# William-Mou/WasmEdge

Measured on AMD Instinct MI355X. Metric: aggregate Wasm instrs/sec at 64K instances, 1/2/4/8 GPUs vs host-core interp, higher is better.
Workload: dtype i32; 1 GPU; C2 BLAKE3 compression loop (configs[1]); instances_per_gpu=65536, instances=65536, parallelism=instance-sharded, 1 process per GPU, compiled_runs=11, engine=compiled-runs+simt/vgpr-frames, granule=4, iters=1000

## Files before the change

### wasmedge_amd/csrc/batch_kernel.hip

```cpp
#include <hip/hip_runtime.h>
#include <stdint.h>

#include <mutex>
#include <vector>

#include "dbc.h"
#include "kparams.h"


#include "dbc_ops.h"
#include "tc.h"
#include "tc_slots.h"

extern "C" __global__ void wb_tc_holder_kernel() {
  asm volatile("s_endpgm\n"
#include "tc_blob.inc"
               ::: "s60", "s61", "s62", "s63", "s64", "s65", "s66", "s67", "s68", "s69",
               "s70", "s71", "s72", "s73", "s74", "s75", "s76", "s77", "s78", "s79", "s80",
               "s81", "s82", "s83", "s84", "s85", "s86", "s87", "s88", "s89", "s90", "s91",
               "s92", "s93", "s94", "s95", "v104", "v105", "v106", "v107", "v108", "v109", "v110", "v111",
               "v112", "v113", "v114", "v115", "v116", "v117", "v118", "v119", "v120",
               "v121", "v122", "v123", "v124", "v125", "v126", "v127", "vcc", "memory");
}
extern "C" __global__ void __launch_bounds__(256) wb_vf_holder_kernel() {
// ... 124 lines not shown
      "v_mov_b32 v105, %[pages]\n\t" \
      "v_mov_b32 v106, %[mlo]\n\t" \
      "v_mov_b32 v107, %[mhi]\n\t" \
      "v_mov_b32 v102, %[gsp]\n\t" \
      "v_mov_b32 v101, %[hwm]\n\t" \
      "v_mov_b32 v103, %[stk]\n\t" \
      "v_mov_b32 v99, %[msh]\n\t" \
      "v_add_u32_e32 v100, 6, v99\n\t" \
      "v_mov_b32 v92, %[vpc]\n\t" \
      "v_mov_b32 v93, 0\n\t" \
      "s_mov_b32 s93, %[slds]\n\t" \
      "v_mov_b32 v94, %[llo]\n\t" \
      "v_mov_b32 v95, %[lhi]\n\t" \
      "v_mov_b32 v96, %[glo]\n\t" \
      "v_mov_b32 v97, %[ghi]\n\t" \
      "s_mov_b32 s94, %[vsync]\n\t" \
      "s_mov_b32 s95, %[low]\n\t" \
      "s_mov_b32 s98, %[xlo]\n\t" \
      "s_mov_b32 s99, %[xhi]\n\t" \
      "s_mov_b64 exec, s[96:97]\n\t" \
      "s_getpc_b64 s[66:67]\n" \
      "Ltc_ret_%=:\n\t" \
      "s_add_u32 s66, s66, Ltc_back_%= - Ltc_ret_%=\n\t" \
      "s_addc_u32 s67, s67, 0\n\t" \
      "s_getpc_b64 s[68:69]\n\t" \
      "s_add_u32 s68, s68, wb_vf_entry@rel32@lo+4\n\t" \
      "s_addc_u32 s69, s69, wb_vf_entry@rel32@hi+12\n\t" \
      "s_setpc_b64 s[68:69]\n" \
      "Ltc_back_%=:\n\t" \
      "s_lshr_b32 %[npc], s62, 5\n\t" \
      "s_mov_b32 %[cnt], s65\n\t" \
      "s_mov_b32 %[why], s92\n\t" \
      "s_mov_b32 %[noth], s63\n\t" \
      "s_mov_b32 %[nlow], s95\n\t" \
      "s_mov_b64 %[ngrp], s[74:75]\n\t" \
      "v_mov_b32 %[gsp], v102\n\t" \
      "v_mov_b32 %[glo], v96\n\t" \
      "v_mov_b32 %[ghi], v97\n\t" \
      "v_mov_b32 %[vpc], v92\n\t" \
      "v_mov_b32 %[vcnt], v93\n\t" \
      "v_mov_b32 %[hwm], v101\n\t" \
      "s_mov_b64 exec, %[ex]" \
       \
      : [npc] "=&s"(npc), [cnt] "=&s"(cnt), [why] "=&s"(why), [noth] "=&s"(noth), [nlow] "=&s"(nlow), \
        [ngrp] "=&s"(ngrp), [gsp] "+v"(gsp), [hwm] "+v"(hwm), [glo] "+v"(glo), [ghi] "+v"(ghi), \
        [vpc] "+v"(vpc), [vcnt] "=&v"(vcnt) \
      : [clo] "s"(clo), [chi] "s"(chi), [pc] "s"(pc), [oth] "s"(oth), [lim] "s"(lim), [fr] "v"(fr), \
        [pages] "v"(pages), [mlo] "v"(mlo), [mhi] "v"(mhi), [stk] "v"(stk), [msh] "s"(msh), \
        [slds] "s"(slds), [vsync] "s"(vsync), [low] "s"(lw), [llo] "s"(llo), [lhi] "s"(lhi), \
        [all] "s"(all), [grp] "s"(grp), [ex] "s"(ex), [xlo] "s"(xlo), [xhi] "s"(xhi) \
      : "s60", "s61", "s62", "s63", "s64", "s65", "s66", "s67", "s68", "s69", "s70", "s71", \
        "s72", "s73", "s74", "s75", "s76", "s77", "s78", "s79", "s80", "s81", "s82", "s83", \
        "s84", "s85", "s86", "s87", "s88", "s89", "s90", "s91", "s92", "s93", "s94", "s95", "s96", "s97", \
        "s98", "s99", \
        "v92", "v93", "v94", "v98", "v95", "v96", "v97", "v99", "v100", "v101", "v102", "v103", "v104", "v105", "v106", "v107", "v108", "v109", "v110", "v111", "v112", "v113", \
        "v114", "v115", "v116", "v117", "v118", "v119", "v120", "v121", "v122", "v123", \
        "v124", "v125", "v126", "v127", "vcc", "scc", "memory", ##__VA_ARGS__);
#define TC_VREGS "v128", "v129", "v130", "v131", "v132", "v133", "v134", "v135", "v136", "v137", \
  "v138", "v139", "v140", "v141", "v142", "v143", "v144", "v145", "v146", "v147", "v148", "v149", \
  "v150", "v151", "v152", "v153", "v154", "v155", "v156", "v157", "v158", "v159", "v160", "v161", \
  "v162", "v163", "v164", "v165", "v166", "v167", "v168", "v169", "v170", "v171", "v172", "v173", \
  "v174", "v175", "v176", "v177", "v178", "v179", "v180", "v181", "v182", "v183", "v184", "v185", \
  "v186", "v187", "v188", "v189", "v190", "v191", "v192", "v193", "v194", "v195", "v196", "v197", \
  "v198", "v199", "v200", "v201", "v202", "v203", "v204", "v205", "v206", "v207", "v208", "v209", \
  "v210", "v211", "v212", "v213", "v214", "v215", "v216", "v217", "v218", "v219", "v220", "v221", \
  "v222", "v223", "v224", "v225", "v226", "v227", "v228", "v229", "v230", "v231", "v232", "v233", \
  "v234", "v235", "v236", "v237", "v238", "v239", "v240", "v241", "v242", "v243", "v244", "v245", \
  "v246", "v247", "v248", "v249", "v250", "v251", "v252", "v253", "v254", "v255"
struct SimtOut {
  uint64_t grp;
  uint32_t oth, low, vpc, vcnt;
};
template <bool VF>
__device__ __forceinline__ uint32_t tc_run(const void *tcode, uint32_t pc, uint32_t other, uint32_t low,
                                           uint32_t fr, uint32_t pages, const uint32_t *mem, uint32_t g,
                                           uint32_t &gsp, uint32_t &hwm, uint32_t stk, uint32_t slds,
                                           uint32_t vsync, uint64_t &gas, uint64_t gas_limit,
                                           uint32_t *ncnt, uint32_t *reason, uint32_t lim,
                                           SimtOut *so = nullptr, uint64_t all = 0, uint64_t grp = 0,
                                           uint32_t vpc = 0, uint64_t xbase = 0) {
  uint32_t npc, cnt, why;
  uint32_t glo = (uint32_t)gas, ghi = (uint32_t)(gas >> 32);
  const uint32_t llo = __builtin_amdgcn_readfirstlane((uint32_t)gas_limit);
  const uint32_t lhi = __builtin_amdgcn_readfirstlane((uint32_t)(gas_limit >> 32));
  const uint32_t oth = __builtin_amdgcn_readfirstlane(other >= (1u << 26) ? 0xFFFFFFFFu : other << 5);
  const uint32_t lw = __builtin_amdgcn_readfirstlane(low >= (1u << 26) ? 0xFFFFFFFFu : low << 5);
  const uint64_t m = (uint64_t)(uintptr_t)mem;
  const uint32_t msh = 2u + g;
  const uint32_t mlo = (uint32_t)m, mhi = (uint32_t)(m >> 32);
  const uint64_t cp = (uint64_t)(uintptr_t)tcode;
  const uint32_t clo = (uint32_t)cp, chi = (uint32_t)(cp >> 32);
  pc = __builtin_amdgcn_readfirstlane(pc);
  if constexpr (VF) {
    const uint64_t ex = __builtin_amdgcn_read_exec();
    if (!so) all = grp = ex;
    const uint32_t xlo = __builtin_amdgcn_readfirstlane((uint32_t)xbase);
    const uint32_t xhi = __builtin_amdgcn_readfirstlane((uint32_t)(xbase >> 32));
    uint32_t noth, nlow, vcnt;
    uint64_t ngrp;
    TC_RUN_VF_ASM(TC_VREGS);
    if (so) *so = SimtOut{ngrp, noth, nlow, vpc, vcnt};
  } else {
    TC_RUN_ASM("wb_tc_entry");
  }
  gas = (uint64_t)glo | ((uint64_t)ghi << 32);
  *ncnt = cnt;
  *reason = why;
// ... 832 lines not shown
```

### wasmedge_amd/csrc/jit.cpp

```cpp
#include "jit.h"

#include <algorithm>
#include <cctype>
#include <cstdarg>
#include <cstdio>
#include <cstdlib>
#include <functional>
#include <map>

#include "frontend.h"
#include "jit_int.h"
#include "tc_slots.h"

namespace wb {
using namespace jit;

namespace {

constexpr uint32_t kMinRun = 3;
constexpr uint32_t kMaxRun = 1500;
constexpr uint32_t kMaxBrTable = 32;

const char *const PAGES = "v105", *const MEM = "v[106:107]", *const HWM = "v101";
const char *const A0 = "v108", *const A1 = "v109", *const AP = "v[108:109]";
const char *const B0 = "v110", *const B1 = "v111", *const BP = "v[110:111]";
const char *const R0 = "v114", *const R1 = "v115", *const RP = "v[114:115]";
const char *const W0 = "v116", *const WP = "v[116:117]";
const char *const X0 = "v118", *const X1 = "v119", *const XP = "v[118:119]";
const char *const Y0 = "v120", *const Y1 = "v121";
const char *const Z0 = "v126", *const Z1 = "v127", *const ZP = "v[126:127]";
const char *const T2 = "s[74:75]";

uint16_t op_of(const DInstr &I) { return uint16_t(I.w0 & 0x7FFFu); }

bool is_store_op(uint16_t op) {
  return op == OP_ST8 || op == OP_ST16 || op == OP_ST32 || op == OP_ST64 || op == OP_ST128;
}

uint32_t mem_bytes(uint16_t op) {
  switch (op) {
    case OP_LD8S32: case OP_LD8U32: case OP_LD8S64: case OP_LD8U64: case OP_ST8: return 1;
    case OP_LD16S32: case OP_LD16U32: case OP_LD16S64: case OP_LD16U64: case OP_ST16: return 2;
    case OP_LD32: case OP_LD32S64: case OP_LD32U64: case OP_ST32: return 4;
    case OP_LD64: case OP_ST64: return 8;
    case OP_LD128: case OP_ST128: return 16;
    default: return 0;
  }
}

bool load_wide_op(uint16_t op) {
  return op == OP_LD8S64 || op == OP_LD8U64 || op == OP_LD16S64 || op == OP_LD16U64 ||
         op == OP_LD32S64 || op == OP_LD32U64 || op == OP_LD64;
}
uint16_t xmop(const DInstr &I) {
  const uint16_t op = uint16_t(I.w0 & 0x7FFFu);
  return op == OP_XLD || op == OP_XST ? uint16_t(I.w2 >> 16) : uint16_t(0);
}
bool is_xfer(uint16_t op) { return op == OP_CALL || op == OP_RET; }
bool is_branch_op(uint16_t op) {
  return op == OP_JMP || op == OP_BR_IF || op == OP_BR_UNLESS || (op >= OP_BR_EQ && op <= OP_BR_GE_U_I);
}
bool ends_run(uint16_t op) { return is_xfer(op) || is_branch_op(op) || op == OP_BR_TABLE || op == OP_TAIL_CALL; }

struct JitTarget {
  const Program &P;
  uint32_t glog;
  const JitCost *cost;
  const std::vector<uint32_t> *xinfo;
  uint32_t xlog;
  uint32_t mem_pages;
};

struct RunIndex {
  std::map<uint32_t, size_t> start;
  std::map<uint32_t, uint32_t> fentry;
  uint32_t ncode;
  RunIndex(const Program &P, const std::vector<JitRun> &runs) : ncode(uint32_t(P.code.size())) {
    for (size_t k = 0; k < runs.size(); k++) start.emplace(runs[k].pc, k);
    for (uint32_t f = 0; f < P.funcs.size(); f++)
      if (!P.funcs[f].imported) fentry[P.funcs[f].entry_pc] = f;
  }
  bool has(uint32_t pc) const { return start.count(pc) != 0; }
  size_t at(uint32_t pc) const { return start.find(pc)->second; }
  int64_t func_of(uint32_t pc) const {
// ... 3425 lines not shown
  return fp;
}

bool jit::recursive(const Program &P) {
  const RunIndex ix(P, {});
  auto func_of = [&](uint32_t pc) { return ix.func_of(pc); };
  const size_t nf = P.funcs.size();
  std::vector<std::vector<uint32_t>> g(nf);
  for (uint32_t pc = 0; pc < P.code.size(); pc++) {
    const uint16_t o = op_of(P.code[pc]);
    if (o == OP_CALL_INDIRECT || o == OP_TAIL_CALL_INDIRECT) return true;
    if (o != OP_CALL && o != OP_TAIL_CALL) continue;
    const int64_t a = func_of(pc), b = func_of(P.code[pc].w3);
    if (a < 0 || b < 0) continue;
    if (a == b) return true;
    g[size_t(a)].push_back(uint32_t(b));
  }
  std::vector<uint8_t> st(nf, 0);
  std::function<bool(uint32_t)> dfs = [&](uint32_t f) -> bool {
    st[f] = 1;
    for (uint32_t t : g[f]) {
      if (st[t] == 1) return true;
      if (st[t] == 0 && dfs(t)) return true;
    }
    st[f] = 2;
    return false;
  };
  for (uint32_t f = 0; f < nf; f++)
    if (st[f] == 0 && dfs(f)) return true;
  return false;
}

JitKnobs jit::read_knobs() {
  auto on = [](const char *name) {
    const char *v = getenv(name);
    return !(v && v[0] == '0');
  };
  JitKnobs k;
  k.hybrid = on("WB_HYBRID");
  k.nanobs = on("WB_NANOBS");
  k.fold = on("WB_FOLD");
  k.cmpany = on("WB_CMPANY");
  k.jit_sched = on("WB_JIT_SCHED");
  k.sched_stores = on("WB_SCHED_STORES");
  k.load_batch = on("WB_LOAD_BATCH");
  k.depth = on("WB_DEPTH");
  k.inline_calls = on("WB_INLINE");
  k.fwd = on("WB_FWD");
  k.fwd_store = on("WB_FWD_STORE");
  k.fwd_alias = on("WB_FWD_ALIAS");
  k.kprop = on("WB_KPROP");
  k.fwd_lazy = on("WB_FWD_LAZY");
  k.fwd_loop = on("WB_FWD_LOOP");
  k.ret_pf = on("WB_RET_PF");
  k.brt_thread = on("WB_BRT_THREAD");
  k.trip_fwd = on("WB_TRIP_FWD");
  k.trip_fwdchk = on("WB_TRIP_FWDCHK");
  k.trip_mad = on("WB_TRIP_MAD");
  k.trip_split = on("WB_TRIP_SPLIT");
  k.trip_pf = on("WB_TRIP_PF");
  k.trip_x4 = on("WB_TRIP_X4");
  k.trip_scanbf = on("WB_TRIP_SCANBF");
  k.trip_batch = on("WB_TRIP_BATCH");
  k.trip_inline = on("WB_TRIP_INLINE");
  k.trip_smask = on("WB_TRIP_SMASK");
  k.trip_cmpbr = on("WB_TRIP_CMPBR");
  k.trip_chain = on("WB_TRIP_CHAIN");
  k.trip_guard = on("WB_TRIP_GUARD");
  const char *c1 = getenv("WB_TRIP_CONV1");
  k.trip_conv1 = c1 && c1[0] == '1';
  const char *sxe = getenv("WB_SIMT_X");
  k.simt_x = sxe ? unsigned(atoi(sxe)) : 7u;
  const char *tse = getenv("WB_TRIP_SCAN");
  k.trip_scan = tse ? std::min<uint32_t>(uint32_t(atoi(tse)), kTripScan) : kTripScan;
  const char *cpe = getenv("WB_TRIP_CONVP");
  k.trip_convp = cpe ? std::min(8u, std::max(1u, uint32_t(atoi(cpe)))) : 4u;
  const char *ose = getenv("WB_TRIP_OUTSH");
  k.trip_outsh = ose ? std::max(0, std::min(6, atoi(ose))) : 6;
  k.nanobs_list = getenv("WB_NANOBS_LIST");
  return k;
}

namespace {

struct SimtPlan {
  std::vector<std::vector<uint64_t>> live;
  std::map<uint32_t, std::vector<uint32_t>> ret_sites;
  std::vector<int64_t> inl_f, inl_post;
  std::map<size_t, FwdPlan> plans;
  std::map<size_t, size_t> loop_of;
  std::vector<std::pair<size_t, int>> jobs;
  std::vector<uint8_t> inl_target;
};

static void inline_of(const JitTarget &t, const JitKnobs &kn, const RunIndex &ix,
                      const std::vector<JitRun> &runs, size_t k, int64_t *inl_f, int64_t *inl_post) {
  const Program &P = t.P;
  *inl_f = *inl_post = -1;
  const JitRun &r = runs[k];
  const DInstr &last = P.code[r.pc + r.len - 1];
  const uint32_t tgt = last.w3, cpc = r.pc + r.len - 1;
  if (op_of(last) != OP_CALL || t.cost || !kn.inline_calls || !ix.has(tgt)) return;
  const JitRun &rf = runs[ix.at(tgt)];
  const uint32_t L = last.w1 & 0xFFFFu, fb = P.global_cells;
  const uint32_t off = L - fb;
  const uint32_t fend = ix.func_end(tgt);
// ... 47 lines not shown
  const RunIndex &ix;
  const std::vector<JitRun> &runs;
  const SimtPlan &pl;
  const std::vector<uint8_t> &nob;
  unsigned sx;
  bool hybrid, depth_pick;
};

struct RunCompile {
  const JitTarget &t;
  const JitKnobs &kn;
  const RunIndex &ix;
  const std::vector<JitRun> &runs;
  const SimtPlan &pl;
  const Program &P;
  const JitCost *const cost;
  const std::vector<uint8_t> &nob;
  const std::vector<std::vector<uint64_t>> &live;
  const unsigned sx;
  const bool hybrid, depth_pick;
  const size_t k;
  const int var;
  const JitRun &r;
  const std::string K, xs;
  const DInstr &last;
  const uint16_t lop;
  const uint32_t fall, tgt;
  bool preload = false;
  Em e;
  uint64_t c_fall = 0;
  int64_t c_adj = 0;
  std::string extra;
  uint32_t fuse_cell = ~0u;
  bool cmp_any = false;
  int lab = 0, nfast = 0;
  size_t head_stubs = 0;

  RunCompile(const SimtCtx &c, size_t k_, int var_)
      : t(c.t), kn(c.kn), ix(c.ix), runs(c.runs), pl(c.pl), P(c.t.P), cost(c.t.cost), nob(c.nob),
        live(c.pl.live), sx(c.sx), hybrid(c.hybrid), depth_pick(c.depth_pick), k(k_), var(var_),
        r(c.runs[k_]), K(std::to_string(k_) + (var_ == 1 ? "c" : var_ == 2 ? "p" : "")), xs("Lxs" + K),
        last(P.code[r.pc + r.len - 1]), lop(op_of(last)), fall(r.pc + r.len),
        tgt((lop == OP_CALL || lop == OP_TAIL_CALL || is_branch_op(lop)) ? last.w3 : 0),
        e(c.t, uint32_t(k_ + size_t(var_) * 2 * c.runs.size()), c.nob.empty() ? nullptr : &c.nob) {
    e.kprop = kn.kprop;
    auto lo = pl.loop_of.find(k);
    const size_t R = var == 2 && lo != pl.loop_of.end() ? lo->second : k;
    auto fp = pl.plans.find(R);
    if (fp != pl.plans.end() && (var != 2 || lo != pl.loop_of.end())) {
      loop = &fp->second;
      lazy = kn.fwd_lazy && kn.fwd_store && var != 0 && !loop->dirty.empty();
      tight = kn.fwd_loop;
      if (tight && var == 2) pre_cnt = runs[R].cnt + runs[size_t(pl.inl_f[R])].cnt;
    }
  }

  const FwdPlan *loop = nullptr;
  bool lazy = false, tight = false;
  uint32_t pre_cnt = 0;
  std::string cold, callee_cold;

  std::string flush_dirty() const {
    if (!lazy) return "";
    Em d(t);
    uint32_t a0 = 0;
    bool open = false;
    for (uint32_t A : loop->dirty) {
      const uint32_t fr = loop->freg.at(A);
      if (t.glog == 0) {
        if (!open || uint64_t(A - a0) * 64u > 4095) {
          d.l("v_mov_b32 %s, 0x%x", W0, A);
          d.l("v_lshlrev_b64 v[122:123], 6, %s", WP);
          d.l("v_lshl_add_u64 v[122:123], v[122:123], 0, %s", MEM);
          a0 = A;
          open = true;
        }
        d.l("global_store_dword v[122:123], v%u, off offset:%u", fr, (A - a0) * 64u);
      } else {
        d.l("v_mov_b32 %s, 0x%x", Y0, A);
        granule_addr(d, XP, Y0, MEM);
        d.l("global_store_dword %s, v%u, off", XP, fr);
      }
    }
    return d.o;
  }

  const char *copy_sfx(size_t q) const {
    auto it = pl.loop_of.find(k);
    return var == 2 && it != pl.loop_of.end() && it->second == q ? "c" : "";
  }

  void entry() {
    e.ret_pf = kn.ret_pf && !cost && !pl.inl_target[k] && ret_prefetch_run(P, r);
    e.l(".p2align 6");
    e.l("Lb%s:", K.c_str());
    const uint32_t pre = lop == OP_CALL || lop == OP_TAIL_CALL ? tgt : fall;
    preload = lop != OP_RET && lop != OP_JMP && lop != OP_BR_TABLE && !ix.has(pre);
    if (preload) {
      e.l("s_waitcnt lgkmcnt(0)");
      e.l("s_mov_b32 s68, 0x%x", pre * 32u);
      e.l("s_load_dwordx8 s[76:83], s[60:61], s68");
      e.l("s_load_dwordx8 s[84:91], s[60:61], s68 offset:0x20");
    }
    if (cost) {
      e.metered = true;
      for (uint32_t i = 0; i < r.len; i++) c_fall += cost->full(P, r.pc + i);
      if (is_branch_op(lop)) c_adj = cost->taken(tgt, int32_t(int16_t(last.w2 >> 16)));
      const uint64_t c_max = c_adj > 0 ? c_fall + uint64_t(c_adj) : c_fall;
      e.pc = r.pc;
      e.l("s_mov_b32 s68, 0x%x", uint32_t(c_max));
      e.l("s_mov_b32 s69, 0x%x", uint32_t(c_max >> 32));
      e.l("v_lshl_add_u64 %s, v[96:97], 0, s[68:69]", XP);
      e.l("v_cmp_gt_u64_e64 %s, %s, v[94:95]", T2, XP);
// ... 77 lines not shown
      if (!ok_emit) return false;
      e.done += (I.w0 >> 16) & 0xFFu;
      if (cost) e.cdone += cost->full(P, r.pc + i);
      if (i == 0 && op_of(I) == OP_POST_CALL) {
        e.l("Lpa%s:", K.c_str());
        head_stubs = e.stubs.size();
      }
    }
    e.def_flush(pl.inl_f[k] >= 0 ? 128 + (last.w1 & 0xFFFFu) : ~0u);
    e.drain();
    if (kn.jit_sched) e.o = e.o.substr(0, body_at) + schedule(e.o.substr(body_at), kn);
    if (tight && var == 2) {
      e.o = e.o.substr(e.o.find("Lpa" + K + ":\n"));
      e.stubs.erase(e.stubs.begin(), e.stubs.begin() + long(head_stubs));
    }
    e.pc = r.pc + r.len - 1;
    e.group = nullptr;
    return true;
  }

  void go(uint32_t to, bool banks) {
    auto it = ix.start.find(to);
    const std::string disp = "Ld" + K + "_" + std::to_string(lab++);
    if (it != ix.start.end()) {
      e.l("s_add_u32 s68, s62, 0x%x", (runs[it->second].len - 1) * 32u);
      e.l("s_cmp_ge_u32 s68, s63");
      e.l("s_cbranch_scc1 %s", disp.c_str());
      const std::string q = "Lq" + K + "_" + std::to_string(lab);
      const std::string tl = "Lb" + std::to_string(it->second) +
                             copy_sfx(it->second);
      long_jump(e, tl, q);
      e.l("%s:", disp.c_str());
      e.o += flush_dirty();
      banks = false;
    }
    e.l("s_waitcnt lgkmcnt(0)");
    if (!banks) {
      e.l("s_load_dwordx8 s[76:83], s[60:61], s62");
      e.l("s_load_dwordx8 s[84:91], s[60:61], s62 offset:0x20");
      e.l("s_waitcnt lgkmcnt(0)");
    }
    e.l("s_add_u32 s68, s70, s76");
    e.l("s_addc_u32 s69, s71, 0");
    e.l("s_setpc_b64 s[68:69]");
  }
  void taken_checks() {
    e.l("s_cmp_ge_u32 s65, s64");
    e.l("s_cbranch_scc1 %s", xs.c_str());
    e.l("s_cmp_le_u32 s62, s95");
    e.l("s_cselect_b32 s63, s95, s63");
    e.l("s_cmp_ge_u32 s62, s63");
    e.l("s_cbranch_scc1 %s", xs.c_str());
  }
  void fast_to(uint32_t to, bool taken, bool lim) {
    auto it = ix.start.find(to);
    if (it == ix.start.end()) return;
    const uint32_t tend = (to + runs[it->second].len - 1) * 32u;
    const std::string tl = "Lb" + std::to_string(it->second) +
                           copy_sfx(it->second);
    if (lim) {
      e.l("s_cmp_gt_u32 s68, 0x%x", tend);
    } else if (taken) {
      if (to == 0) {
        e.l("s_mov_b32 s63, s95");
      } else {
        e.l("s_cmp_ge_u32 s95, 0x%x", to * 32u);
        e.l("s_cselect_b32 s63, s95, s63");
      }
      e.l("s_cmp_lt_u32 s65, s64");
      e.l("s_cselect_b32 s68, s63, 0");
      e.l("s_cmp_gt_u32 s68, 0x%x", tend);
    } else {
      e.l("s_cmp_gt_u32 s63, 0x%x", tend);
    }
    cond_jump(e, tl, "Lf" + K + "_" + std::to_string(nfast++));
  }
  void fallthrough(uint32_t cnt) {
    e.gas_add(c_fall);
    e.l("s_add_u32 s65, s65, 0x%x", cnt + pre_cnt);
    fast_to(fall, false, false);
    e.l("s_mov_b32 s62, 0x%x", fall * 32u);
    e.l("s_cmp_ge_u32 s62, s63");
    e.l("s_cbranch_scc1 %s", xs.c_str());
    go(fall, preload);
  }

  bool tail_inlined() {
    const int64_t inl_f = pl.inl_f[k], inl_post = pl.inl_post[k];
    const auto fwd_it = pl.plans.find(k);
    const FwdPlan *fwd = fwd_it != pl.plans.end() ? &fwd_it->second : nullptr;
    const JitRun &rf = runs[size_t(inl_f)];
    const uint32_t L = last.w1 & 0xFFFFu, nargs = last.w1 >> 16, nloc = last.w2 & 0xFFFFu;
    const uint32_t fb = P.global_cells, off = L - fb, n = L - fb, callpc = e.pc;
    const std::string IK = "i" + K;
    if (!(tight && var == 1)) {
      e.l("v_add_u32_e32 %s, %u, v102", X0, n + 1);
      e.l("v_cmp_lt_u32_e64 %s, s93, %s", T2, X0);
      e.leave_if_t2();
    }
    const std::vector<uint8_t> dead = dead_zeros(P, rf);
    Em ei = e.inlined(e.run + uint32_t(runs.size()), off, r.cnt);
    ei.kprop = e.kprop;
    ei.def.swap(e.def);
    for (uint32_t q = 0; q < nloc; q++)
      if (dead.empty() || !dead[fb + nargs + q]) {
        if (ei.kprop) prop_const(ei, fb + nargs + q, 0);
        else ei.l("v_mov_b32 %s, 0", ei.v(fb + nargs + q));
      }
    std::vector<int> lead2;
    const std::vector<MemGroup> groups2 = jit_groups(P, rf, &lead2);
    const size_t body2 = ei.o.size();
    const bool fc = fwd && var == 1;
// ... 116 lines not shown
          }
          out += ln + "\n";
        }
        if (written) {
          ei.o = ei.o.substr(0, mark) + out;
          ei.amap.erase(dx.first);
        } else {
          ei.o.resize(mark);
          ei.materialize(dx.first);
          if (!emit(ei, I)) return false;
        }
      }
      deferred.clear();
      if (fa >= 0 && op_of(I) == OP_ST32) {
        ei.before_write(fwd->freg.at(uint32_t(fa)));
        ei.l("v_mov_b32 v%u, %s", fwd->freg.at(uint32_t(fa)), ei.v(I.w1 >> 16));
      }
      if (fa >= 0 && fwd->copy_now[i]) {
        ei.sync({I.w2 & 0xFFFFu});
        ei.l("v_mov_b32 v%u, %s", fwd->freg.at(uint32_t(fa)), ei.v(I.w2 & 0xFFFFu));
      }
      ei.done += (I.w0 >> 16) & 0xFFu;
    }
    ei.drain();
    if (fwd && !fc)
      for (const auto &fc2 : fwd->end_copy) ei.l("v_mov_b32 v%u, v%u", fc2.first, 128 + fc2.second);
    ei.group = nullptr;
    if (kn.jit_sched) ei.o = ei.o.substr(0, body2) + schedule(ei.o.substr(body2), kn);
    const DInstr &rt = P.code[rf.pc + rf.len - 1];
    const uint32_t ra = rt.w1 & 0xFFFFu, nres = rt.w1 >> 16;
    ei.def_flush(128 + L);
    for (uint32_t q = 0; q < nres; q++) {
      const std::string from = ei.sv(ra + q);
      ei.before_write(128 + L + q);
      ei.def.erase(128 + L + q);
      ei.l("v_mov_b32 v%u, %s", 128 + L + q, from.c_str());
    }
    ei.amap.clear();
    ei.def.clear();
    if (!(tight && fwd)) ei.l("s_add_u32 s65, s65, 0x%x", r.cnt + rf.cnt);
    {
      const JitRun &rp = runs[size_t(inl_post)];
      const DInstr &pl = P.code[rp.pc + rp.len - 1];
      const uint16_t plo = op_of(pl);
      const uint32_t ptgt = (plo == OP_CALL || is_branch_op(plo)) ? pl.w3 : 0;
      const uint32_t ppre = plo == OP_CALL ? ptgt : rp.pc + rp.len;
      if (plo != OP_RET && plo != OP_JMP && plo != OP_BR_TABLE && !ix.has(ppre)) {
        ei.l("s_waitcnt lgkmcnt(0)");
        ei.l("s_mov_b32 s68, 0x%x", ppre * 32u);
        ei.l("s_load_dwordx8 s[76:83], s[60:61], s68");
        ei.l("s_load_dwordx8 s[84:91], s[60:61], s68 offset:0x20");
      }
    }
    ei.l("s_mov_b32 s62, 0x%x", (callpc + 1) * 32u);
    if (!(tight && var == 1))
      long_jump(ei, "Lpa" + std::to_string(inl_post) + (fwd ? "p" : ""), "Lpq" + IK);
    std::string deopt;
    {
      Em d(t);
      d.l("s_waitcnt vmcnt(0)");
      d.l("v_lshl_add_u32 %s, v102, 8, v103", X1);
      for (uint32_t q = 0; q < n; q++) d.l("ds_write_b32 %s, v%u offset:%u", X1, 128 + fb + q, q * 256u);
      d.l("v_mov_b32 %s, 0x%x", Y1, ((callpc + 1) & 0xFFFFFu) | (L << 20));
      d.l("ds_write_b32 %s, %s offset:%u", X1, Y1, n * 256u);
      d.l("v_add_u32_e32 v102, %u, v102", n + 1);
      for (uint32_t c = fb; c < P.total_cells(); c++) d.l("v_mov_b32 v%u, v%u", 128 + c, 128 + c + off);
      deopt = d.o;
    }
    e.l("Li%s:", IK.c_str());
    e.o += ei.o;
    ei.o = ei.tail;
    for (const auto &st : ei.stubs) {
      ei.o += st.lab + ":\n" + st.fix + flush_dirty() + deopt;
      ei.l("s_mov_b32 s62, 0x%x", st.pc * 32u);
      ei.l("s_add_u32 s65, s65, 0x%x", st.done);
      ei.l("s_setpc_b64 s[70:71]");
    }
    callee_cold = ei.o;
    return true;
  }
  void tail_tail_call() {
    std::vector<uint8_t> dead;
    if (ix.has(tgt)) dead = dead_zeros(P, runs[ix.at(tgt)]);
    emit_tail_call(e, last, dead.empty() ? nullptr : &dead);
    e.gas_add(c_fall);
    e.l("s_add_u32 s65, s65, 0x%x", r.cnt);
    fast_to(tgt, true, false);
    e.l("s_mov_b32 s62, 0x%x", tgt * 32u);
    taken_checks();
    go(tgt, preload);
  }
  void tail_call() {
    std::vector<uint8_t> dead;
    if (ix.has(tgt)) dead = dead_zeros(P, runs[ix.at(tgt)]);
    emit_call(e, last, e.pc, dead.empty() ? nullptr : &dead);
    e.gas_add(c_fall);
    e.l("s_add_u32 s65, s65, 0x%x", r.cnt);
    fast_to(tgt, true, false);
    e.l("s_mov_b32 s62, 0x%x", tgt * 32u);
    taken_checks();
    go(tgt, preload);
  }
  void tail_ret() {
    std::vector<uint32_t> sites;
    const int64_t f = ix.func_of(e.pc);
    const auto rs_it = f >= 0 ? pl.ret_sites.find(uint32_t(f)) : pl.ret_sites.end();
    if (rs_it != pl.ret_sites.end())
      for (uint32_t rs : rs_it->second)
        if (ix.has(rs) && sites.size() < 6) sites.push_back(rs);
    std::vector<std::pair<uint32_t, std::string>> known;
    for (size_t q = 0; q < sites.size() && q < 2 && !cost; q++) {
      const DInstr &cl = P.code[sites[q] - 1];
      const uint32_t L = cl.w1 & 0xFFFFu;
      if (op_of(cl) == OP_CALL && L < 4096)
        known.push_back({(sites[q] & 0xFFFFFu) | (L << 20), "Lrk" + K + "_" + std::to_string(q)});
    }
    const std::string rout = emit_ret(e, last, (sx & 2) ? "Lrs" + K : std::string(), known);
    if (sx & 2) {
      const uint32_t a = last.w1 & 0xFFFFu, nres = last.w1 >> 16, fb = e.fb;
      Em x(t);
      x.l("Lrs%s:", K.c_str());
      x.l("v_and_b32_e32 %s, 0xfffff, %s", X0, Y1);
      x.l("v_cmp_eq_u32_e32 vcc, 0xfffff, %s", X0);
      x.l("s_and_b64 vcc, vcc, exec");
      x.l("s_cbranch_vccnz %s", rout.c_str());
      x.l("v_subrev_u32_e32 v102, 1, v102");
// ... 42 lines not shown
      fast_to(sites[q], true, true);
      taken_checks();
      e.l("Lrt%s_%zu:", K.c_str(), q);
      go(sites[q], false);
    }
    for (size_t q = 0; q < known.size(); q++) {
      const uint32_t a = last.w1 & 0xFFFFu, nres = last.w1 >> 16, fb = e.fb;
      e.l("%s:", known[q].second.c_str());
      e.l("v_subrev_u32_e32 v102, 1, v102");
      for (uint32_t c = 0; c < nres; c++)
        if (a != fb) e.l("v_mov_b32 %s, %s", e.V(fb + c).c_str(), e.V(a + c).c_str());
      e.l("s_add_u32 s65, s65, 0x%x", r.cnt);
      fast_to(sites[q], true, false);
      e.l("s_mov_b32 s62, 0x%x", sites[q] * 32u);
      taken_checks();
      go(sites[q], false);
    }
  }
  void tail_br_table() {
    emit_br_table(e, last);
    e.l("v_readfirstlane_b32 s68, %s", Y0);
    e.l("v_readfirstlane_b32 s69, %s", Y1);
    e.l("s_nop 1");
    e.l("v_cmp_ne_u32_e64 %s, s68, %s", T2, Y0);
    e.l("v_cmp_ne_u32_e32 vcc, s69, %s", Y1);
    e.l("s_or_b64 %s, %s, vcc", T2, T2);
    e.l("s_and_b64 %s, %s, exec", T2, T2);
    if (sx & 1) {
      e.l("s_cbranch_scc1 Lts%s", K.c_str());
      Em x(t);
      x.l("Lts%s:", K.c_str());
      x.l("v_mov_b32 %s, %s", VPC, Y0);
      x.l("v_add_u32_e32 %s, %s, %s", VCNT, VCNT, Y1);
      x.l("s_add_u32 s65, s65, 0x%x", r.cnt);
      flush(x);
      long_jump(x, "Lsched", "Ltq" + K);
      extra += x.o;
    } else {
      const std::string lab_split = "Lx" + K + "_" + std::to_string(e.stubs.size());
      e.stubs.push_back(Em::Stub{lab_split, e.pc, e.done, e.cdone, e.def_fix()});
      e.l("s_cbranch_scc1 %s", lab_split.c_str());
    }
    e.l("s_lshl_b32 s62, s68, 5");
    e.l("s_add_u32 s65, s65, 0x%x", r.cnt);
    e.l("s_add_u32 s65, s65, s69");
    taken_checks();
    go(~0u, false);
  }
  void tail_branch() {
    const uint32_t bcnt = (last.w0 >> 16) & 0xFFu;
    const int32_t tcnt = int32_t(int16_t(last.w2 >> 16));
    const uint32_t taken_cnt = uint32_t(int32_t(r.cnt) + tcnt);
    const std::string nt = "Lnt" + K;
    if (lop != OP_JMP) {
      if (cmp_any) {
        if (lop == OP_BR_UNLESS) e.l("s_not_b64 vcc, vcc");
      } else {
        if (fuse_cell != ~0u) {
          e.alias_cell = int64_t(fuse_cell);
          e.alias_reg = 114;
        }
        branch_cond(e, last);
        e.alias_cell = -1;
      }
      e.l("s_and_b64 %s, vcc, exec", T2);
      e.l("s_cbranch_scc0 %s", nt.c_str());
      e.l("s_cmp_eq_u64 %s, exec", T2);
      if (sx & 1) {
        e.l("s_cbranch_scc0 Lbs%s", K.c_str());
        Em x(t);
        x.l("Lbs%s:", K.c_str());
        x.o += flush_dirty();
        {
          auto inl = [](int64_t v) { return v >= -16 && v <= 64; };
          std::string f = std::to_string(fall), t = std::to_string(tgt);
          if (!inl(fall)) { x.l("v_mov_b32 %s, 0x%x", X0, fall); f = X0; }
          if (!inl(tgt)) { x.l("v_mov_b32 %s, 0x%x", X1, tgt); t = X1; }
          x.l("v_cndmask_b32_e64 %s, %s, %s, vcc", VPC, f.c_str(), t.c_str());
          if (inl(tcnt)) {
            x.l("v_cndmask_b32_e64 %s, 0, %d, vcc", X0, int32_t(tcnt));
          } else {
            x.l("v_mov_b32 %s, 0x%x", X1, uint32_t(tcnt));
            x.l("v_cndmask_b32_e32 %s, 0, %s, vcc", X0, X1);
          }
          x.l("v_add_u32_e32 %s, %s, %s", VCNT, VCNT, X0);
        }
        x.l("s_add_u32 s65, s65, 0x%x", r.cnt + pre_cnt);
        flush(x);
        if (fall != tgt && !hybrid && !depth_pick) {
          const uint32_t lo = std::min(fall, tgt), hi = std::max(fall, tgt);
          x.l("s_cmp_le_u32 s95, 0x%x", lo * 32u);
          x.l("s_cbranch_scc0 Lbf%s", K.c_str());
          long_jump(x, "Lsched", "Lbq" + K);
          x.l("Lbf%s:", K.c_str());
          x.l("s_sub_u32 s64, s64, 16");
          x.l("s_cselect_b32 s64, 0, s64");
          x.l("s_cmp_eq_u32 s95, -1");
          x.l("s_cbranch_scc0 Lbm%s", K.c_str());
          x.l("s_add_u32 s70, s70, 0x%x", 2u * TC_BANK_BYTES);
          x.l("s_addc_u32 s71, s71, 0");
          x.l("s_add_u32 s72, s70, 0x%x", TC_BANK_BYTES);
          x.l("s_addc_u32 s73, s71, 0");
          x.l("Lbm%s:", K.c_str());
          x.l("s_min_u32 s95, s95, 0x%x", hi * 32u);
          x.l("s_mov_b32 s63, s95");
          x.l(lo == tgt ? "s_and_b64 s[74:75], vcc, exec" : "s_andn2_b64 s[74:75], exec, vcc");
          x.l("s_mov_b32 s62, 0x%x", lo * 32u);
          x.l("s_waitcnt lgkmcnt(0)");
          x.l("s_load_dwordx8 s[76:83], s[60:61], s62");
          x.l("s_load_dwordx8 s[84:91], s[60:61], s62 offset:0x20");
          long_jump(x, "Lsc_disp", "Lbt" + K);
        } else {
          long_jump(x, "Lsched", "Lbq" + K);
        }
        extra += x.o;
      } else {
        const std::string lab_split = "Lx" + K + "_" + std::to_string(e.stubs.size());
        e.stubs.push_back(Em::Stub{lab_split, e.pc, e.done, e.cdone, e.def_fix()});
        e.l("s_cbranch_scc0 %s", lab_split.c_str());
      }
    }
    e.gas_add(uint64_t(int64_t(c_fall) + c_adj));
    e.l("s_add_u32 s65, s65, 0x%x", taken_cnt + pre_cnt);
    fast_to(tgt, true, false);
    e.l("s_mov_b32 s62, 0x%x", tgt * 32u);
    taken_checks();
    go(tgt, false);
    if (lop != OP_JMP) {
      e.l("%s:", nt.c_str());
      (void)bcnt;
      e.o += flush_dirty();
      fallthrough(r.cnt);
    }
  }

  void finish() {
    const size_t hot = e.o.size();
    e.l("Lxs%s:", K.c_str());
    e.o += flush_dirty();
    if (sx & 4) {
      long_jump(e, "Lmerge", "Lmq" + K);
    } else {
      e.l("s_add_u32 s68, s70, %u", TC_JIT_XS);
      e.l("s_addc_u32 s69, s71, 0");
      e.l("s_setpc_b64 s[68:69]");
    }
    e.o += extra;
    e.o += e.tail;
    for (const auto &s : e.stubs) {
      e.l("%s:", s.lab.c_str());
      e.o += s.fix;
      e.o += flush_dirty();
      e.gas_add(s.cdone);
      e.l("s_mov_b32 s62, 0x%x", s.pc * 32u);
      e.l("s_add_u32 s65, s65, 0x%x", s.done + pre_cnt);
      e.l("s_setpc_b64 s[70:71]");
    }
    if (tight && var == 1) {
      cold = callee_cold + e.o.substr(hot);
      e.o.resize(hot);
    } else {
      e.o.insert(hot, callee_cold);
    }
  }

  bool compile() {
    entry();
    if (!body()) return false;
    if (pl.inl_f[k] >= 0) {
      if (!tail_inlined()) return false;
    } else if (lop == OP_TAIL_CALL) {
      tail_tail_call();
    } else if (lop == OP_CALL) {
      tail_call();
    } else if (lop == OP_RET) {
      tail_ret();
    } else if (lop == OP_BR_TABLE) {
      tail_br_table();
    } else if (is_branch_op(lop)) {
      tail_branch();
    } else {
      fallthrough(r.cnt);
    }
    finish();
    return true;
  }
};

}

std::string jit_source(const Program &P, const std::vector<JitRun> &runs, uint32_t glog,
                       const JitCost *cost, bool simt, bool trip, const std::vector<uint32_t> *xinfo,
                       uint32_t xlog, uint32_t mem_pages) {
  if (cost) simt = false;
  if (!P.xmems.empty() && (!xinfo || xinfo->size() < 2 * P.xmems.size())) return "";
  const JitKnobs kn = read_knobs();
  const JitTarget t{P, glog, cost, xinfo, xlog, mem_pages};
  const RunIndex ix(P, runs);
  const bool trips = trip && simt && runs.size() <= kTripMaxRuns;
  const bool hybrid = trips && kn.hybrid;
  if (trips && !hybrid) return trip_source(t, kn, ix, runs, false);
  const std::vector<uint8_t> nob = kn.nanobs ? nan_observable(P, kn) : std::vector<uint8_t>();
  const SimtPlan pl = plan_simt(t, kn, ix, runs);
  const unsigned sx = simt ? kn.simt_x : 0u;
  std::string body;
// ... 83 lines not shown
```

### wasmedge_amd/csrc/jit_int.h

```cpp
#pragma once
#include <cstdint>
#include <string>

#include "jit.h"

namespace wb {
namespace jit {

constexpr uint32_t kMadPages = 1000;
constexpr uint32_t kTripScan = 4;

struct JitKnobs {
  bool hybrid;
  bool nanobs;
  bool fold;
  bool cmpany;
  bool jit_sched;
  bool sched_stores;
  bool load_batch;
  bool depth;
  bool inline_calls;
  bool fwd;
  bool fwd_store;
  bool fwd_alias;
  bool kprop;
  bool fwd_lazy;
  bool fwd_loop;
  bool ret_pf;
  bool brt_thread;
  bool trip_fwd;
  bool trip_fwdchk;
  bool trip_mad;
  bool trip_split;
  bool trip_pf;
  bool trip_x4;
  bool trip_scanbf;
  bool trip_batch;
  bool trip_inline;
  bool trip_smask;
  bool trip_cmpbr;
  bool trip_chain;
  bool trip_guard;
  bool trip_conv1;
  unsigned simt_x;
  uint32_t trip_scan;
  uint32_t trip_convp;
  int trip_outsh;
  const char *nanobs_list;
};
JitKnobs read_knobs();

std::string schedule(const std::string &body, const JitKnobs &kn);
std::string resolve_jumps(const std::string &body);

bool recursive(const Program &P);

}
}
```

Baseline: 132700 billion instr/s.

## Hoist loop budget check into precomputed trip counter for tight forwarded loops

Adds a scalar trip counter (s100) for tight forwarded loops. On loop entry it computes how many whole iterations fit in the remaining instruction budget and pre-charges the count. When the whole wave takes the back-edge, it decrements this counter instead of doing the per-trip budget compare and count update. All exit paths (stubs, side exits, divergence) refund the unused pre-charged count. This removes scalar bookkeeping from the back-edge of hot loops such as the BLAKE3 round loop, at the cost of more exit-path code and a new clobbered SGPR.

Measured after the change: 136000 billion instr/s, median of 6. +2.5%, better.

```diff
diff --git a/wasmedge_amd/csrc/batch_kernel.hip b/wasmedge_amd/csrc/batch_kernel.hip
--- a/wasmedge_amd/csrc/batch_kernel.hip
+++ b/wasmedge_amd/csrc/batch_kernel.hip
@@ -200,7 +200,7 @@
       : "s60", "s61", "s62", "s63", "s64", "s65", "s66", "s67", "s68", "s69", "s70", "s71", \
         "s72", "s73", "s74", "s75", "s76", "s77", "s78", "s79", "s80", "s81", "s82", "s83", \
         "s84", "s85", "s86", "s87", "s88", "s89", "s90", "s91", "s92", "s93", "s94", "s95", "s96", "s97", \
-        "s98", "s99", \
+        "s98", "s99", "s100", \
         "v92", "v93", "v94", "v98", "v95", "v96", "v97", "v99", "v100", "v101", "v102", "v103", "v104", "v105", "v106", "v107", "v108", "v109", "v110", "v111", "v112", "v113", \
         "v114", "v115", "v116", "v117", "v118", "v119", "v120", "v121", "v122", "v123", \
         "v124", "v125", "v126", "v127", "vcc", "scc", "memory", ##__VA_ARGS__);
diff --git a/wasmedge_amd/csrc/jit.cpp b/wasmedge_amd/csrc/jit.cpp
--- a/wasmedge_amd/csrc/jit.cpp
+++ b/wasmedge_amd/csrc/jit.cpp
@@ -30,6 +30,7 @@
 const char *const Y0 = "v120", *const Y1 = "v121";
 const char *const Z0 = "v126", *const Z1 = "v127", *const ZP = "v[126:127]";
 const char *const T2 = "s[74:75]";
+const char *const TRIPS = "s100";
 
 uint16_t op_of(const DInstr &I) { return uint16_t(I.w0 & 0x7FFFu); }
 
@@ -3561,6 +3562,7 @@
   k.kprop = on("WB_KPROP");
   k.fwd_lazy = on("WB_FWD_LAZY");
   k.fwd_loop = on("WB_FWD_LOOP");
+  k.fwd_tail = k.fwd_loop && on("WB_FWD_TAIL");
   k.ret_pf = on("WB_RET_PF");
   k.brt_thread = on("WB_BRT_THREAD");
   k.trip_fwd = on("WB_TRIP_FWD");
@@ -3714,13 +3716,29 @@
       lazy = kn.fwd_lazy && kn.fwd_store && var != 0 && !loop->dirty.empty();
       tight = kn.fwd_loop;
       if (tight && var == 2) pre_cnt = runs[R].cnt + runs[size_t(pl.inl_f[R])].cnt;
+      const JitRun &rp = runs[loop->post];
+      const DInstr &br = P.code[rp.pc + rp.len - 1];
+      if (tight && kn.fwd_tail && op_of(br) != OP_JMP) {
+        hoist = true;
+        trip_cnt = uint32_t(int32_t(rp.cnt) + int32_t(int16_t(br.w2 >> 16))) + runs[R].cnt +
+                   runs[size_t(pl.inl_f[R])].cnt;
+      }
     }
   }
 
   const FwdPlan *loop = nullptr;
-  bool lazy = false, tight = false;
-  uint32_t pre_cnt = 0;
+  bool lazy = false, tight = false, hoist = false;
+  uint32_t pre_cnt = 0, trip_cnt = 0;
   std::string cold, callee_cold;
+
+  std::string cnt_fix() const {
+    if (!hoist || var == 0) return "";
+    Em d(t);
+    d.l("s_mul_i32 s68, %s, 0x%x", TRIPS, trip_cnt);
+    d.l("s_sub_u32 s65, s65, s68");
+    d.l("s_mov_b32 %s, 0", TRIPS);
+    return d.o;
+  }
 
   std::string flush_dirty() const {
     if (!lazy) return "";
@@ -3904,12 +3922,12 @@
     e.l("s_cmp_ge_u32 s62, s63");
     e.l("s_cbranch_scc1 %s", xs.c_str());
   }
-  void fast_to(uint32_t to, bool taken, bool lim) {
+  void fast_to(uint32_t to, bool taken, bool lim, const std::string &via = std::string()) {
     auto it = ix.start.find(to);
     if (it == ix.start.end()) return;
     const uint32_t tend = (to + runs[it->second].len - 1) * 32u;
-    const std::string tl = "Lb" + std::to_string(it->second) +
-                           copy_sfx(it->second);
+    const std::string tl = !via.empty() ? via : "Lb" + std::to_string(it->second) +
+                                                    copy_sfx(it->second);
     if (lim) {
       e.l("s_cmp_gt_u32 s68, 0x%x", tend);
     } else if (taken) {
@@ -4132,7 +4150,8 @@
         ei.l("s_load_dwordx8 s[84:91], s[60:61], s68 offset:0x20");
       }
     }
-    ei.l("s_mov_b32 s62, 0x%x", (callpc + 1) * 32u);
+    if (!(hoist && fwd && var == 1)) ei.l("s_mov_b32 s62, 0x%x", (callpc + 1) * 32u);
+    if (hoist && fwd && var == 0) ei.l("s_mov_b32 %s, 0", TRIPS);
     if (!(tight && var == 1))
       long_jump(ei, "Lpa" + std::to_string(inl_post) + (fwd ? "p" : ""), "Lpq" + IK);
     std::string deopt;
@@ -4151,7 +4170,7 @@
     e.o += ei.o;
     ei.o = ei.tail;
     for (const auto &st : ei.stubs) {
-      ei.o += st.lab + ":\n" + st.fix + flush_dirty() + deopt;
+      ei.o += st.lab + ":\n" + st.fix + flush_dirty() + deopt + cnt_fix();
       ei.l("s_mov_b32 s62, 0x%x", st.pc * 32u);
       ei.l("s_add_u32 s65, s65, 0x%x", st.done);
       ei.l("s_setpc_b64 s[70:71]");
@@ -4300,6 +4319,8 @@
     const int32_t tcnt = int32_t(int16_t(last.w2 >> 16));
     const uint32_t taken_cnt = uint32_t(int32_t(r.cnt) + tcnt);
     const std::string nt = "Lnt" + K;
+    const bool hoisted = hoist && var == 2 && lop != OP_JMP && ix.has(tgt);
+    const std::string head = hoisted ? "Lb" + std::to_string(ix.at(tgt)) + copy_sfx(ix.at(tgt)) : "";
     if (lop != OP_JMP) {
       if (cmp_any) {
         if (lop == OP_BR_UNLESS) e.l("s_not_b64 vcc, vcc");
@@ -4310,6 +4331,25 @@
         }
         branch_cond(e, last);
         e.alias_cell = -1;
+      }
+      if (hoisted) {
+        e.l("s_cmp_eq_u64 vcc, exec");
+        e.l("s_cbranch_scc0 Lsl%s", K.c_str());
+        e.l("s_add_u32 %s, %s, -1", TRIPS, TRIPS);
+        cond_jump(e, head, "Lft" + K);
+        e.l("s_mov_b32 %s, 0", TRIPS);
+        e.l("Lsl%s:", K.c_str());
+        e.o += cnt_fix();
+        Em x(t);
+        x.l("Lhd%s:", K.c_str());
+        x.l("s_sub_u32 s68, s64, s65");
+        x.l("s_sub_u32 s68, s68, 1");
+        x.l("s_mul_hi_u32 %s, s68, 0x%x", TRIPS,
+            uint32_t(std::min<uint64_t>(0xFFFFFFFFull, (1ull << 32) / trip_cnt)));
+        x.l("s_mul_i32 s68, %s, 0x%x", TRIPS, trip_cnt);
+        x.l("s_add_u32 s65, s65, s68");
+        long_jump(x, head, "Lhq" + K);
+        extra += x.o;
       }
       e.l("s_and_b64 %s, vcc, exec", T2);
       e.l("s_cbranch_scc0 %s", nt.c_str());
@@ -4370,7 +4410,7 @@
     }
     e.gas_add(uint64_t(int64_t(c_fall) + c_adj));
     e.l("s_add_u32 s65, s65, 0x%x", taken_cnt + pre_cnt);
-    fast_to(tgt, true, false);
+    fast_to(tgt, true, false, hoisted ? "Lhd" + K : std::string());
     e.l("s_mov_b32 s62, 0x%x", tgt * 32u);
     taken_checks();
     go(tgt, false);
@@ -4386,6 +4426,7 @@
     const size_t hot = e.o.size();
     e.l("Lxs%s:", K.c_str());
     e.o += flush_dirty();
+    e.o += cnt_fix();
     if (sx & 4) {
       long_jump(e, "Lmerge", "Lmq" + K);
     } else {
@@ -4399,6 +4440,7 @@
       e.l("%s:", s.lab.c_str());
       e.o += s.fix;
       e.o += flush_dirty();
+      e.o += cnt_fix();
       e.gas_add(s.cdone);
       e.l("s_mov_b32 s62, 0x%x", s.pc * 32u);
       e.l("s_add_u32 s65, s65, 0x%x", s.done + pre_cnt);
diff --git a/wasmedge_amd/csrc/jit_int.h b/wasmedge_amd/csrc/jit_int.h
--- a/wasmedge_amd/csrc/jit_int.h
+++ b/wasmedge_amd/csrc/jit_int.h
@@ -26,6 +26,7 @@
   bool kprop;
   bool fwd_lazy;
   bool fwd_loop;
+  bool fwd_tail;
   bool ret_pf;
   bool brt_thread;
   bool trip_fwd;
```
